# SrikarK-code/clip-dplm

Measured on AMD Instinct MI355X. Metric: seq-pairs/sec/node, contrastive training step, ESM-2-35M dual encoder, higher is better.
Workload: dtype bf16

## Files before the change

### clip_dplm_amd/_ffi.py

```python
from __future__ import annotations

import ctypes as C
import os

_HERE = os.path.dirname(os.path.abspath(__file__))
LIB_PATH = os.path.join(_HERE, "lib", "libclipk.so")

BF16, F32, U8 = 0, 1, 2
SAME_CLASS = {"mask": 0, "positive": 1}
ACT_NONE, ACT_RELU, ACT_GELU, ACT_CELU, ACT_SOFTPLUS = 0, 1, 2, 3, 4
ACT = {None: ACT_NONE, "none": ACT_NONE, "relu": ACT_RELU, "gelu": ACT_GELU, "celu": ACT_CELU, "softplus": ACT_SOFTPLUS}


class ClipkError(RuntimeError):
    pass


class GemmArgs(C.Structure):
    _fields_ = [
        ("A", C.c_void_p), ("lda", C.c_int64),
        ("B", C.c_void_p), ("ldb", C.c_int64),
        ("C", C.c_void_p), ("ldc", C.c_int64), ("c_dtype", C.c_int),
        ("M", C.c_int), ("N", C.c_int), ("K", C.c_int),
        ("bias", C.c_void_p),
        ("act", C.c_int),
        ("out_preact", C.c_void_p), ("ldp", C.c_int64),
        ("dact_aux", C.c_void_p), ("ldd", C.c_int64),
        ("dact", C.c_int),
        ("residual", C.c_void_p), ("ldr", C.c_int64), ("r_dtype", C.c_int),
        ("alpha", C.c_float),
        ("drop_p", C.c_float), ("drop_seed", C.c_uint32),
        ("rope_cos", C.c_void_p), ("rope_sin", C.c_void_p),
        ("rope_L", C.c_int), ("rope_hd", C.c_int), ("rope_cols", C.c_int), ("rope_row0", C.c_int),
        ("aux_dtype", C.c_int),
        ("rope_interleaved", C.c_int),
    ]


_vp, _i, _i64, _f, _sz = C.c_void_p, C.c_int, C.c_int64, C.c_float, C.c_size_t

SIGNATURES = {
    "clipk_version": (_i, []),
    "clipk_arch": (C.c_char_p, []),
    "clipk_status_string": (C.c_char_p, [_i]),
    "clipk_set_option": (_i, [C.c_char_p, _i]),
    "clipk_get_option": (_i, [C.c_char_p, C.POINTER(_i)]),
    "clipk_reset_options": (_i, []),
    "clipk_gemm_nt": (_i, [C.POINTER(GemmArgs), _vp]),
    "clipk_gemm_wgrad_workspace": (_sz, [_i, _i, _i]),
    "clipk_gemm_wgrad": (_i, [_vp, _i64, _vp, _i64, _vp, _i64, _vp, _i, _i, _i, _i, _i, _i, _vp, _sz, _vp]),
    "clipk_simce_workspace": (_sz, [_i, _i, _i]),
    "clipk_simce_lse": (_i, [_vp, _i, _vp, _i, _vp, _i, _i, _vp, _i, _vp, _vp, _vp, _sz, _vp]),
    "clipk_simce_grad": (_i, [_vp, _i, _vp, _i, _vp, _i, _i, _vp, _i, _vp, _vp, _f, _f, _f, _vp, _vp, _vp, _sz, _vp]),
    "clipk_simce_grad_scaled": (_i, [_vp, _i, _vp, _i, _vp, _i, _i, _vp, _i, _vp, _vp, _f, _f, _f, _vp, _vp, _vp, _vp, _sz, _vp]),
    "clipk_ce_combine": (_i, [_vp, _vp, _vp, _vp, _i, _f, _f, _f, _vp, _vp]),
    "clipk_simce_cls_workspace": (_sz, [_i, _i, _i]),
    "clipk_simce_lse_cls": (_i, [_vp, _i, _vp, _i, _vp, _i, _i, _vp, _i, _vp, _vp, _i, _f, _vp, _vp, _vp, _vp, _sz, _vp]),
    "clipk_simce_grad_cls": (_i, [_vp, _i, _vp, _i, _vp, _i, _i, _vp, _i, _vp, _vp, _vp, _vp, _vp, _vp, _i, _f, _i, _f, _f,
                                  _f, _vp, _vp, _vp, _vp, _sz, _vp]),
    "clipk_simce_hard_workspace": (_sz, [_i, _i, _i]),
    "clipk_simce_lse_hard": (_i, [_vp, _i, _vp, _i, _vp, _i, _i, _vp, _f, _i, _vp, _vp, _vp, _vp, _vp, _vp, _sz, _vp]),
    "clipk_simce_grad_hard": (_i, [_vp, _i, _vp, _i, _vp, _i, _i, _vp, _f, _i, _vp, _vp, _vp, _vp, _f, _f, _f, _vp, _vp,
                                   _vp, _vp, _sz, _vp]),
    "clipk_simce_pairs_workspace": (_sz, [_i, _i, _i]),
    "clipk_simce_lse_pairs": (_i, [_vp, _i, _i, _i, C.POINTER(_i), _i, _vp, _vp, _vp, _vp, _sz, _vp]),
    "clipk_simce_grad_pairs": (_i, [_vp, _i, _i, _i, C.POINTER(_i), C.POINTER(_i), _i, _vp, _vp, _f, _f, _f, _vp, _vp,
                                    _vp, _sz, _vp]),
    "clipk_simce_pairs_cls_workspace": (_sz, [_i, _i, _i]),
    "clipk_simce_lse_pairs_cls": (_i, [_vp, _i, _i, _i, C.POINTER(_i), _i, _vp, C.POINTER(_vp), _i, _f, _vp, _vp, _vp, _vp,
                                       _sz, _vp]),
    "clipk_simce_grad_pairs_cls": (_i, [_vp, _i, _i, _i, C.POINTER(_i), C.POINTER(_i), _i, _vp, C.POINTER(_vp), _i, _f, _vp,
                                        _vp, _f, _f, _f, _vp, _vp, _vp, _vp, _sz, _vp]),
    "clipk_simce_pairs_hard_workspace": (_sz, [_i, _i, _i]),
    "clipk_simce_lse_pairs_hard": (_i, [_vp, _i, _i, _i, C.POINTER(_i), _i, _vp, _f, C.POINTER(_vp), _vp, _vp, _vp, _vp,
                                        _sz, _vp]),
    "clipk_simce_grad_pairs_hard": (_i, [_vp, _i, _i, _i, C.POINTER(_i), C.POINTER(_i), _i, _vp, _f, C.POINTER(_vp), _vp,
                                         _f, _f, _f, _vp, _vp, _vp, _vp, _sz, _vp]),
    "clipk_sim_logits": (_i, [_vp, _i, _vp, _i, _i, _vp, _vp, _i64, _vp]),
    "clipk_sim_topk_workspace": (_sz, [_i, _i, _i, _i]),
    "clipk_sim_topk": (_i, [_vp, _i, _vp, _i, _i, _f, _i, _vp, _vp, _vp, _sz, _vp]),
    "clipk_sim_knn_workspace": (_sz, [_i, _i, _i, _i]),
    "clipk_sim_knn": (_i, [_vp, _i, _vp, _i, _i, _f, _vp, _i64, _vp, _vp, _i, _vp, _vp, _vp, _sz, _vp]),
# ... 140 lines not shown
```

### clip_dplm_amd/csrc/common.h

```cpp
#pragma once
#include <hip/hip_runtime.h>
#include <stdint.h>
#include "../../include/clipk.h"

#define CLIPK_ABI_VERSION 7
#define WAVE 64

enum clipk_opt {
  OPT_GEMM_KERNEL = 0,
  OPT_GEMM_EPI_GENERIC,
  OPT_GEMM_BM,
  OPT_GEMM_STAGES,
  OPT_GEMM_NWG,
  OPT_GEMM_STAGGER,
  OPT_EPI_NT,
  OPT_WGRAD_KERNEL,
  OPT_ATTN_WHOLE_FWD,
  OPT_ATTN_FUSED_BWD,
  OPT_ATTN_FUSED_WAVES,
  OPT_WGRAD_SPLITS,
  OPT_SIMCE_KERNEL,
  OPT_ATTN_ROW_STORES,
  OPT_GEMM_F32_SPLITS,
  OPT_RETRIEVAL_SPLITS,
  OPT_COUNT
};
int clipk_opt_get(int which);

typedef __attribute__((ext_vector_type(8))) short bf16x8;
typedef __attribute__((ext_vector_type(4))) short bf16x4;
typedef __attribute__((ext_vector_type(4))) float f32x4;
typedef __attribute__((ext_vector_type(16))) float f32x16;
typedef __attribute__((ext_vector_type(4))) unsigned int u32x4;
typedef __attribute__((ext_vector_type(2))) unsigned int u32x2;

__device__ __forceinline__ float bf16_to_f32(unsigned short h) {
  return __uint_as_float(((unsigned int)h) << 16);
}
__device__ __forceinline__ unsigned short f32_to_bf16(float f) {
  __bf16 b = (__bf16)f;
  return __builtin_bit_cast(unsigned short, b);
}
__device__ __forceinline__ unsigned int pack_bf16x2(float lo, float hi) {
  typedef __attribute__((ext_vector_type(2))) float v2f;
  typedef __attribute__((ext_vector_type(2))) __bf16 v2b;
  const v2b v = __builtin_convertvector(v2f{lo, hi}, v2b);
  return __builtin_bit_cast(unsigned int, v);
}

__device__ __forceinline__ void gelu_parts(float x, float& erf_abs, float& e) {
  const float ax = fabsf(x);
  const float t = __builtin_amdgcn_rcpf(fmaf(0.3275911f * 0.70710678118654752440f, ax, 1.0f));
  e = __builtin_amdgcn_exp2f(-0.72134752044448170368f * x * x);
  float poly = fmaf(1.061405429f, t, -1.453152027f);
  poly = fmaf(poly, t, 1.421413741f);
  poly = fmaf(poly, t, -0.284496736f);
  poly = fmaf(poly, t, 0.254829592f);
// ... 197 lines not shown
```

### clip_dplm_amd/csrc/core.hip

```cpp
#include "common.h"

extern "C" int clipk_version(void) { return CLIPK_ABI_VERSION; }
extern "C" const char* clipk_arch(void) { return "gfx950"; }
extern "C" const char* clipk_status_string(int status) {
  switch (status) {
    case CLIPK_OK: return "ok";
    case CLIPK_ERR_BAD_ARG: return "bad argument (null / misaligned pointer or non-positive dimension)";
    case CLIPK_ERR_UNSUPPORTED: return "unsupported shape for the gfx950 kernels";
    case CLIPK_ERR_LAUNCH: return "HIP launch error";
    default: return "unknown clipk status";
  }
}

#include <atomic>
#include <string.h>
namespace {
struct OptDef { const char* name; int dflt; };
const OptDef kOpts[OPT_COUNT] = {
    {"gemm_kernel", -1}, {"gemm_epi_generic", 0}, {"gemm_bm", 0}, {"gemm_stages", 1}, {"gemm_nwg", 0},
    {"gemm_stagger", 0}, {"epi_nt", 0}, {"wgrad_kernel", -1}, {"attn_whole_fwd", -1}, {"attn_fused_bwd", -1},
    {"attn_fused_waves", 0}, {"wgrad_splits", 0}, {"simce_kernel", -1},
    {"attn_row_stores", 0}, {"gemm_f32_splits", 0}, {"retrieval_splits", 0},
};
std::atomic<int> g_opts[OPT_COUNT];
std::atomic<bool> g_opts_init{false};
void opts_init() {
  if (!g_opts_init.load(std::memory_order_acquire)) {
    for (int i = 0; i < OPT_COUNT; ++i) g_opts[i].store(kOpts[i].dflt, std::memory_order_relaxed);
    g_opts_init.store(true, std::memory_order_release);
  }
}
int opt_index(const char* name) {
  if (!name) return -1;
  for (int i = 0; i < OPT_COUNT; ++i)
    if (strcmp(name, kOpts[i].name) == 0) return i;
  return -1;
}
}

namespace { std::atomic<const unsigned*> g_drop_epoch{nullptr}; }
const unsigned* clipk_drop_epoch() { return g_drop_epoch.load(std::memory_order_relaxed); }
extern "C" int clipk_set_dropout_epoch(const uint32_t* epoch_dev) {
  g_drop_epoch.store(reinterpret_cast<const unsigned*>(epoch_dev), std::memory_order_relaxed);
  return CLIPK_OK;
}

int clipk_opt_get(int which) {
  opts_init();
  return g_opts[which].load(std::memory_order_relaxed);
}
extern "C" int clipk_set_option(const char* name, int value) {
  opts_init();
  const int i = opt_index(name);
  if (i < 0) return CLIPK_ERR_BAD_ARG;
  g_opts[i].store(value, std::memory_order_relaxed);
// ... 15 lines not shown
```

### clip_dplm_amd/csrc/gemm_wgrad.hip

```cpp
#include "common.h"
#include <stdlib.h>

struct clipk_wgrad_v3_args {
  const unsigned short* dY; long lddy;
  const unsigned short* X; long ldx;
  float* slab; float* bslab;
  int M, N, K;
  int ntn, ntk, splits, m_per_split;
};
extern "C" void clipk_wgrad_v3_plan(int M, int N, int K, int* ntn, int* ntk, int* splits, int* mps);
extern "C" int clipk_wgrad_v3_launch(const clipk_wgrad_v3_args* a, void* stream);

namespace {

constexpr int BN = 128, BKO = 128, BMS = 64, NTHREADS = 256;
constexpr int ROWB = 256;
constexpr int TILE_BYTES = BMS * ROWB;
constexpr int LDS_BYTES = 2 * TILE_BYTES;

struct WP {
  const unsigned short* dY; long lddy;
  const unsigned short* X; long ldx;
  float* slab;
  float* bslab;
  int M, N, K;
  int ntn, ntk, splits, m_per_split;
};

typedef __attribute__((ext_vector_type(4))) short s16x4;

__device__ __forceinline__ int seg_off(int row, int seg) { return row * ROWB + ((seg ^ (row & 7)) << 5); }

__device__ __forceinline__ bf16x8 tr_frag(const char* tile, int row0, int seg, int pbyte) {
  const s16x4 lo = __builtin_amdgcn_ds_read_tr16_b64_v4i16(
      (s16x4 __attribute__((address_space(3)))*)(tile + seg_off(row0, seg) + pbyte));
  const s16x4 hi = __builtin_amdgcn_ds_read_tr16_b64_v4i16(
      (s16x4 __attribute__((address_space(3)))*)(tile + seg_off(row0 + 16, seg) + pbyte));
  bf16x8 f;
  f[0] = lo[0]; f[1] = lo[1]; f[2] = lo[2]; f[3] = lo[3];
  f[4] = hi[0]; f[5] = hi[1]; f[6] = hi[2]; f[7] = hi[3];
  return f;
}

// ... 88 lines not shown
      }
      if (do_bias) {
#pragma unroll
        for (int i = 0; i < 4; ++i) accb[i] = __builtin_amdgcn_mfma_f32_16x16x32_bf16(af[i], ones, accb[i], 0, 0, 0);
      }
    }
    __syncthreads();
  }

  float* slab = p.slab + (long)split * p.N * p.K;
#pragma unroll
  for (int i = 0; i < 4; ++i)
#pragma unroll
    for (int j = 0; j < 4; ++j) {
      const int k = k0 + wk * 64 + j * 16 + li;
#pragma unroll
      for (int r = 0; r < 4; ++r) {
        const int n = n0 + wn * 64 + i * 16 + 4 * g + r;
        if (n < p.N && k < p.K) slab[(long)n * p.K + k] = acc[i][j][r];
      }
    }
  if (do_bias && li == 0) {
#pragma unroll
    for (int i = 0; i < 4; ++i)
#pragma unroll
      for (int r = 0; r < 4; ++r) {
        const int n = n0 + wn * 64 + i * 16 + 4 * g + r;
        if (n < p.N) p.bslab[(long)split * p.N + n] = accb[i][r];
      }
  }
}

__global__ void wgrad_reduce_kernel(const float* slab, const float* bslab, int splits, int bsplits, int N, int K,
                                    float* dW, long lddw, float* dbias, int accumulate, int il_hd, int il_rows) {
  const long total4 = (long)N * K / 4;
  const int k4 = K >> 2;
  const long stride = (long)gridDim.x * blockDim.x;
  for (long i = blockIdx.x * (long)blockDim.x + threadIdx.x; i < total4; i += stride) {
    f32x4 a = f32x4{0.f, 0.f, 0.f, 0.f};
    const long sstride = (long)N * K / 4;
    const f32x4* src = reinterpret_cast<const f32x4*>(slab) + i;
    int s = 0;
    for (; s + 8 <= splits; s += 8) {
      f32x4 v[8];
#pragma unroll
      for (int e = 0; e < 8; ++e) v[e] = src[(long)(s + e) * sstride];
      a += (v[0] + v[1]) + (v[2] + v[3]);
      a += (v[4] + v[5]) + (v[6] + v[7]);
    }
    for (; s + 4 <= splits; s += 4) {
      const f32x4 v0 = src[(long)s * sstride], v1 = src[(long)(s + 1) * sstride];
      const f32x4 v2 = src[(long)(s + 2) * sstride], v3 = src[(long)(s + 3) * sstride];
      a += (v0 + v1) + (v2 + v3);
    }
    for (; s < splits; ++s) a += src[(long)s * sstride];
    const long n = i / k4; const int c = (int)(i - n * k4);
    f32x4* o = reinterpret_cast<f32x4*>(dW + (long)il_src((int)n, il_hd, il_rows) * lddw + 4 * c);
    *o = accumulate ? (*o + a) : a;
  }
  if (dbias) {
    for (long i = blockIdx.x * (long)blockDim.x + threadIdx.x; i < N; i += stride) {
      float a = 0.f;
      int s = 0;
      for (; s + 8 <= bsplits; s += 8) {
        float t[8];
#pragma unroll
        for (int e = 0; e < 8; ++e) t[e] = bslab[(long)(s + e) * N + i];
        a += ((t[0] + t[1]) + (t[2] + t[3])) + ((t[4] + t[5]) + (t[6] + t[7]));
      }
      for (; s < bsplits; ++s) a += bslab[(long)s * N + i];
      const int o = il_src((int)i, il_hd, il_rows);
      dbias[o] = accumulate ? dbias[o] + a : a;
    }
  }
}

struct Plan { int ntn, ntk, splits, mps; };
Plan make_plan(int M, int N, int K) {
  Plan pl;
  pl.ntn = (N + BN - 1) / BN; pl.ntk = (K + BKO - 1) / BKO;
  const int ntiles = pl.ntn * pl.ntk;
  int splits = (1024 + ntiles - 1) / ntiles;
  const int max_splits = (M + 8 * BMS - 1) / (8 * BMS);
  if (splits > max_splits) splits = max_splits;
  if (splits < 1) splits = 1;
  int mps = (M + splits - 1) / splits;
  mps = (mps + BMS - 1) / BMS * BMS;
  pl.mps = mps;
  pl.splits = (M + mps - 1) / mps;
  return pl;
}

bool use_v3(int M, int N, int K) {
  const int mode = clipk_opt_get(OPT_WGRAD_KERNEL);
  if (mode == 2) return false;
  if (mode == 3 || mode == 4) return M >= 1024;
  return M >= 16384 && N >= 128 && K >= 128;
}

}

extern "C" size_t clipk_gemm_wgrad_workspace(int M, int N, int K) {
  if (M <= 0 || N <= 0 || K <= 0) return 0;
  const Plan pl = make_plan(M, N, K);
  int ntn, ntk, splits, mps;
  clipk_wgrad_v3_plan(M, N, K, &ntn, &ntk, &splits, &mps);
  const size_t a = (size_t)pl.splits * ((size_t)N * K + N), b = (size_t)splits * ((size_t)N * K + (size_t)ntk * N);
  return (a > b ? a : b) * sizeof(float);
}

extern "C" int clipk_gemm_wgrad(const void* dY, int64_t lddy, const void* X, int64_t ldx,
                                float* dW, int64_t lddw, float* dbias, int M, int N, int K, int accumulate,
                                int il_hd, int il_rows, void* workspace, size_t workspace_bytes, void* stream) {
  if (!dY || !X || !dW || !workspace || M <= 0 || N <= 0 || K <= 0) return CLIPK_ERR_BAD_ARG;
  if (il_rows < 0 || il_rows > N || (il_rows > 0 && (il_hd < 2 || (il_hd & 1) || il_rows % il_hd))) return CLIPK_ERR_BAD_ARG;
  if (il_rows == 0) il_hd = 2;
  if ((N & 7) || (K & 7) || (lddy & 7) || (ldx & 7) || (lddw & 3)) return CLIPK_ERR_UNSUPPORTED;
  if (!aligned16(dY) || !aligned16(X) || !aligned16(dW) || !aligned16(workspace)) return CLIPK_ERR_BAD_ARG;
  hipStream_t st = (hipStream_t)stream;
  if (use_v3(M, N, K)) {
    clipk_wgrad_v3_args a;
    clipk_wgrad_v3_plan(M, N, K, &a.ntn, &a.ntk, &a.splits, &a.m_per_split);
    if (workspace_bytes < (size_t)a.splits * ((size_t)N * K + (size_t)a.ntk * N) * sizeof(float)) return CLIPK_ERR_BAD_ARG;
    a.dY = (const unsigned short*)dY; a.lddy = lddy;
    a.X = (const unsigned short*)X; a.ldx = ldx;
    a.slab = (float*)workspace;
    a.bslab = dbias ? (float*)workspace + (size_t)a.splits * N * K : nullptr;
    a.M = M; a.N = N; a.K = K;
    int rc = clipk_wgrad_v3_launch(&a, stream);
    if (rc) return rc;
    long total4 = (long)N * K / 4;
    int blocks = (int)((total4 + 255) / 256); if (blocks > 2048) blocks = 2048; if (blocks < 1) blocks = 1;
    hipLaunchKernelGGL(wgrad_reduce_kernel, dim3(blocks), dim3(256), 0, st, (const float*)a.slab, (const float*)a.bslab,
                       a.splits, a.splits * a.ntk, N, K, dW, (long)lddw, dbias, accumulate, il_hd, il_rows);
    return clipk_check_launch();
  }
  const Plan pl = make_plan(M, N, K);
  const size_t need = (size_t)pl.splits * ((size_t)N * K + N) * sizeof(float);
  if (workspace_bytes < need) return CLIPK_ERR_BAD_ARG;
  WP p;
  p.dY = (const unsigned short*)dY; p.lddy = lddy;
  p.X = (const unsigned short*)X; p.ldx = ldx;
  p.slab = (float*)workspace;
  p.bslab = dbias ? (float*)workspace + (size_t)pl.splits * N * K : nullptr;
  p.M = M; p.N = N; p.K = K;
  p.ntn = pl.ntn; p.ntk = pl.ntk; p.splits = pl.splits; p.m_per_split = pl.mps;
  hipLaunchKernelGGL(wgrad_kernel, dim3(pl.ntn * pl.ntk * pl.splits), dim3(NTHREADS), LDS_BYTES, st, p);
  int rc = clipk_check_launch();
  if (rc) return rc;
  long total4 = (long)N * K / 4;
  int blocks = (int)((total4 + 255) / 256); if (blocks > 2048) blocks = 2048; if (blocks < 1) blocks = 1;
  hipLaunchKernelGGL(wgrad_reduce_kernel, dim3(blocks), dim3(256), 0, st, (const float*)p.slab, (const float*)p.bslab,
                     pl.splits, pl.splits, N, K, dW, (long)lddw, dbias, accumulate, il_hd, il_rows);
  return clipk_check_launch();
}
```

### clip_dplm_amd/csrc/gemm_wgrad_v3.hip

```cpp
#include "common.h"
#include <stdlib.h>
#include <type_traits>

struct clipk_wgrad_v3_args {
  const unsigned short* dY; long lddy;
  const unsigned short* X; long ldx;
  float* slab;
  float* bslab;
  int M, N, K;
  int ntn, ntk, splits, m_per_split;
};

namespace {

constexpr int BN = 256, BKO = 256, BMS = 64;
constexpr int ROWB = 256;
constexpr int HALF_BYTES = BMS * ROWB;
constexpr int BUF_BYTES = 4 * HALF_BYTES;
constexpr int LDS_BYTES = 2 * BUF_BYTES;
constexpr int YH0 = 0, YH1 = HALF_BYTES, XH0 = 2 * HALF_BYTES, XH1 = 3 * HALF_BYTES;

typedef __attribute__((ext_vector_type(2))) unsigned int u32x2;

template <int OFF>
__device__ __forceinline__ u32x2 ds_tr16(unsigned lds_addr) {
  u32x2 v;
  asm volatile("ds_read_b64_tr_b16 %0, %1 offset:%2" : "=v"(v) : "v"(lds_addr), "n"(OFF));
  return v;
}
template <int OFF>
__device__ __forceinline__ bf16x8 tr_pair(unsigned lds_addr) {
  const u32x2 lo = ds_tr16<OFF>(lds_addr);
  const u32x2 hi = ds_tr16<OFF + 16 * ROWB>(lds_addr);
  const u32x4 f = {lo[0], lo[1], hi[0], hi[1]};
  return __builtin_bit_cast(bf16x8, f);
}

template <int KH, int NH>
__device__ __forceinline__ void quad(f32x4 (&acc)[8][4], const bf16x8 (&yf)[4][2], const bf16x8 (&xf)[2][2][2]) {
#pragma unroll
  for (int ms = 0; ms < 2; ++ms)
#pragma unroll
    for (int u = 0; u < 2; ++u)
#pragma unroll
      for (int t = 0; t < 4; ++t)
        acc[NH * 4 + t][KH * 2 + u] =
            __builtin_amdgcn_mfma_f32_16x16x32_bf16(yf[t][ms], xf[KH][u][ms], acc[NH * 4 + t][KH * 2 + u], 0, 0, 0);
}

#define CLIPK_SB() __builtin_amdgcn_sched_barrier(0)
#define CLIPK_BAR() __builtin_amdgcn_s_barrier()

template <int SCHED>
__global__ __launch_bounds__(512, 1) void wgrad_v3_kernel(const clipk_wgrad_v3_args p) {
  extern __shared__ __attribute__((aligned(16))) char smem[];
  const int tid = threadIdx.x, lane = tid & 63;
  const int wid = __builtin_amdgcn_readfirstlane(tid >> 6);
  const int wn = wid >> 2, wk = wid & 3;
  const int ntiles = p.ntn * p.ntk;
  const int bid = xcd_remap(blockIdx.x, gridDim.x);
  const int split = bid / ntiles;
  const int tile = bid - split * ntiles;
  const int tn = tile / p.ntk, tk = tile - tn * p.ntk;
  const int n0 = tn * BN, k0 = tk * BKO;
  const int M = p.M, N = p.N, K = p.K;
  const int m_beg = split * p.m_per_split;
  int m_end = m_beg + p.m_per_split; m_end = m_end < M ? m_end : M;
  const int nkt = (m_end - m_beg + BMS - 1) / BMS;
  const bool has_bias = p.bslab != nullptr;
  int bias_T = tk;

  unsigned yv[2], xv[2];
#pragma unroll
  for (int i = 0; i < 2; ++i) {
    const int row = 4 * (2 * wid + i) + (lane >> 4);
    const int slot = lane & 15;
    const int col = (((slot >> 1) ^ (row & 7)) << 4) + (slot & 1) * 8;
    yv[i] = (unsigned)(((long)row * p.lddy + (col >> 6) * 128 + (col & 63)) * 2);
    xv[i] = (unsigned)(((long)row * p.ldx + (col >> 5) * 64 + (col & 31)) * 2);
  }
  const unsigned short* y_end = p.dY + ((long)(M - 1) * p.lddy + N);
  const unsigned short* x_end = p.X + ((long)(M - 1) * p.ldx + K);
  auto stage = [&](bool is_y, int half, int T, int region) {
    const long mt = (long)m_beg + (long)T * BMS;
    const unsigned short* base = is_y ? p.dY + mt * p.lddy + (n0 + half * 64) : p.X + mt * p.ldx + (k0 + half * 32);
    const long left = ((is_y ? y_end : x_end) - base) * 2;
    const int bytes = left > 0 ? (int)(left < 0x7fffffffL ? left : 0x7fffffffL) : 0;
    const auto d = __builtin_amdgcn_make_buffer_rsrc((void*)base, 0, bytes, 0x00020000);
    char* dst = smem + (T & 1) * BUF_BYTES + region + wid * 2048;
#pragma unroll
    for (int i = 0; i < 2; ++i)
      __builtin_amdgcn_raw_ptr_buffer_load_lds(d, (__attribute__((address_space(3))) void*)(dst + i * 1024), 16,
                                               (int)(is_y ? yv[i] : xv[i]), 0, 0, 0);
  };
  auto stage1 = [&](bool is_y, int half, int T, int region, int i) {
    const long mt = (long)m_beg + (long)T * BMS;
    const unsigned short* base = is_y ? p.dY + mt * p.lddy + (n0 + half * 64) : p.X + mt * p.ldx + (k0 + half * 32);
    const long left = ((is_y ? y_end : x_end) - base) * 2;
    const int bytes = left > 0 ? (int)(left < 0x7fffffffL ? left : 0x7fffffffL) : 0;
    const auto d = __builtin_amdgcn_make_buffer_rsrc((void*)base, 0, bytes, 0x00020000);
    char* dst = smem + (T & 1) * BUF_BYTES + region + wid * 2048 + i * 1024;
    __builtin_amdgcn_raw_ptr_buffer_load_lds(d, (__attribute__((address_space(3))) void*)dst, 16,
                                             (int)(is_y ? (i ? yv[1] : yv[0]) : (i ? xv[1] : xv[0])), 0, 0, 0);
  };

  f32x4 acc[8][4];
#pragma unroll
  for (int i = 0; i < 8; ++i)
#pragma unroll
    for (int j = 0; j < 4; ++j) acc[i][j] = f32x4{0.f, 0.f, 0.f, 0.f};
  f32x4 accb[2][2];
#pragma unroll
  for (int u = 0; u < 2; ++u) { accb[u][0] = f32x4{0.f, 0.f, 0.f, 0.f}; accb[u][1] = accb[u][0]; }
  bf16x8 ones;
#pragma unroll
  for (int j = 0; j < 8; ++j) ones[j] = (short)0x3F80;

  const int g = lane >> 4, li = lane & 15;
  const int trow = 4 * g + (li >> 2);
  const int sw = trow & 7;
  const unsigned lds0 = (unsigned)(size_t)(__attribute__((address_space(3))) char*)smem;
  unsigned ya[4], xa[2];
#pragma unroll
  for (int t = 0; t < 4; ++t) ya[t] = lds0 + trow * ROWB + (((wn * 4 + t) ^ sw) << 5) + 8 * (li & 3);
#pragma unroll
  for (int u = 0; u < 2; ++u) xa[u] = lds0 + trow * ROWB + (((wk * 2 + u) ^ sw) << 5) + 8 * (li & 3);

  if constexpr (SCHED == 1) {
    bf16x8 yf[4][2], xf[2][2][2];

// ... 76 lines not shown
      CLIPK_SB();
      __builtin_amdgcn_s_setprio(1);
      quad<1, 1>(acc, yf, xf);
      __builtin_amdgcn_s_setprio(0);
      CLIPK_SB(); CLIPK_BAR(); CLIPK_SB();
      if (TM == 0) {
        stage(false, 1, T + 2, XH1);
        asm volatile("s_waitcnt vmcnt(6)" ::: "memory");
      } else if (TM == 1) {
        asm volatile("s_waitcnt vmcnt(0)" ::: "memory");
      }
      CLIPK_SB(); CLIPK_BAR(); CLIPK_SB();
      __builtin_amdgcn_s_setprio(1);
      quad<0, 1>(acc, yf, xf);
      if (bias_now) { bias_tile(accb[1][0], accb[1][1]); bias_T += p.ntk; }
      __builtin_amdgcn_s_setprio(0);
      CLIPK_SB(); CLIPK_BAR(); CLIPK_SB();
    };

    stage(false, 0, 0, XH0); stage(true, 0, 0, YH0); stage(false, 1, 0, XH1); stage(true, 1, 0, YH1);
    if (nkt > 1) {
      stage(false, 0, 1, XH0); stage(true, 0, 1, YH0); stage(false, 1, 1, XH1);
      asm volatile("s_waitcnt vmcnt(6)" ::: "memory");
    } else {
      asm volatile("s_waitcnt vmcnt(0)" ::: "memory");
    }
    CLIPK_SB(); CLIPK_BAR(); CLIPK_SB();
    if (wn == 1) CLIPK_BAR();
    for (int T = 0; T < nkt - 2; ++T) step_body(std::integral_constant<int, 0>{}, T);
    if (nkt > 1) step_body(std::integral_constant<int, 1>{}, nkt - 2);
    step_body(std::integral_constant<int, 2>{}, nkt - 1);
    if (wn == 0) CLIPK_BAR();
  } else {
    bf16x8 yq[2][2][2], xf[2][2][2];
    auto read_yq = [&](auto q_c, unsigned bo) {
      constexpr int q = decltype(q_c)::value;
      constexpr int REG = (q >> 1) ? YH1 : YH0;
#pragma unroll
      for (int t = 0; t < 2; ++t) {
        yq[q & 1][t][0] = tr_pair<REG>(ya[(q & 1) * 2 + t] + bo);
        yq[q & 1][t][1] = tr_pair<REG + 32 * ROWB>(ya[(q & 1) * 2 + t] + bo);
      }
    };
    auto read_x = [&](auto kh_c, unsigned bo) {
      constexpr int kh = decltype(kh_c)::value;
      constexpr int REG = kh ? XH1 : XH0;
#pragma unroll
      for (int u = 0; u < 2; ++u) {
        xf[kh][u][0] = tr_pair<REG>(xa[u] + bo);
        xf[kh][u][1] = tr_pair<REG + 32 * ROWB>(xa[u] + bo);
      }
    };
    auto blk = [&](auto kh_c, auto q_c, auto&& mid) {
      constexpr int kh = decltype(kh_c)::value, q = decltype(q_c)::value;
#pragma unroll
      for (int ms = 0; ms < 2; ++ms) {
#pragma unroll
        for (int u = 0; u < 2; ++u)
#pragma unroll
          for (int t = 0; t < 2; ++t)
            acc[q * 2 + t][kh * 2 + u] = __builtin_amdgcn_mfma_f32_16x16x32_bf16(yq[q & 1][t][ms], xf[kh][u][ms],
                                                                                 acc[q * 2 + t][kh * 2 + u], 0, 0, 0);
        if (ms == 0) { CLIPK_SB(); mid(); CLIPK_SB(); }
      }
    };
    const int b_odd = wk >> 1, b_sel = wk & 1;
    auto bias_mfma = [](int odd, int sel, int qo, f32x4& a0, f32x4& a1, const bf16x8& on, const bf16x8& y00,
                        const bf16x8& y01, const bf16x8& y10, const bf16x8& y11) {
      asm volatile(
          "s_nop 1\n\t"
          "s_cmp_lg_u32 %[odd], %[qo]\n\t"
          "s_cbranch_scc1 2f\n\t"
          "s_cmp_lg_u32 %[sel], 0\n\t"
          "s_cbranch_scc1 1f\n\t"
          "v_mfma_f32_16x16x32_bf16 %[a0], %[y00], %[on], %[a0]\n\t"
          "v_mfma_f32_16x16x32_bf16 %[a1], %[y01], %[on], %[a1]\n\t"
          "s_branch 2f\n"
          "1:\n\t"
          "v_mfma_f32_16x16x32_bf16 %[a0], %[y10], %[on], %[a0]\n\t"
          "v_mfma_f32_16x16x32_bf16 %[a1], %[y11], %[on], %[a1]\n"
          "2:\n\t"
          : [a0] "+v"(a0), [a1] "+v"(a1)
          : [odd] "s"(odd), [sel] "s"(sel), [qo] "s"(qo), [on] "v"(on), [y00] "v"(y00), [y01] "v"(y01),
            [y10] "v"(y10), [y11] "v"(y11)
          : "scc");
    };
#define CLIPK_BIAS_Q(q, a0, a1) \
  bias_mfma(b_odd, b_sel, (q) & 1, a0, a1, ones, yq[(q) & 1][0][0], yq[(q) & 1][0][1], yq[(q) & 1][1][0], yq[(q) & 1][1][1])
    using I0 = std::integral_constant<int, 0>; using I1 = std::integral_constant<int, 1>;
    using I2 = std::integral_constant<int, 2>; using I3 = std::integral_constant<int, 3>;
#define CLIPK_LGKM0() asm volatile("s_waitcnt lgkmcnt(0)" ::: "memory")

    auto step2 = [&](auto mode_c, int T) {
      constexpr int TM = decltype(mode_c)::value;
      const unsigned bo = (T & 1) * BUF_BYTES, bn = ((T + 1) & 1) * BUF_BYTES;
      const bool bias_now = has_bias && T == bias_T;
      const bool y1_next = TM != 2 && T >= 1;
      auto none = [] {};
      CLIPK_LGKM0(); CLIPK_SB();
      read_yq(I1{}, bo); read_x(I1{}, bo);
      CLIPK_SB();
      blk(I0{}, I0{}, [&] { if (y1_next) stage1(true, 1, T + 1, YH1, 0); });
      if (bias_now) CLIPK_BIAS_Q(0, accb[0][0], accb[0][1]);
      CLIPK_SB();
      CLIPK_LGKM0(); CLIPK_SB();
      blk(I1{}, I0{}, [&] { if (y1_next) stage1(true, 1, T + 1, YH1, 1); });
      CLIPK_SB();
      if (TM == 2) asm volatile("s_waitcnt vmcnt(0)" ::: "memory");
      else asm volatile("s_waitcnt vmcnt(8)" ::: "memory");
      CLIPK_SB(); CLIPK_BAR(); CLIPK_SB();
      read_yq(I2{}, bo);
      CLIPK_SB();
      blk(I1{}, I1{}, [&] { if (TM == 0) stage1(true, 0, T + 2, YH0, 0); });
      if (bias_now) CLIPK_BIAS_Q(1, accb[0][0], accb[0][1]);
      CLIPK_SB();
      blk(I0{}, I1{}, [&] { if (TM == 0) stage1(true, 0, T + 2, YH0, 1); });
      CLIPK_SB();
      CLIPK_LGKM0(); CLIPK_SB();
      read_yq(I3{}, bo);
      CLIPK_SB();
      blk(I0{}, I2{}, [&] { if (TM == 0) stage1(false, 0, T + 2, XH0, 0); });
      if (bias_now) CLIPK_BIAS_Q(2, accb[1][0], accb[1][1]);
      CLIPK_SB();
      blk(I1{}, I2{}, [&] { if (TM == 0) stage1(false, 0, T + 2, XH0, 1); });
      CLIPK_SB();
      CLIPK_LGKM0();
      if (TM == 0) asm volatile("s_waitcnt vmcnt(6)" ::: "memory");
      else if (TM == 1) asm volatile("s_waitcnt vmcnt(2)" ::: "memory");
      CLIPK_SB(); CLIPK_BAR(); CLIPK_SB();
      if (TM != 2) read_yq(I0{}, bn);
      CLIPK_SB();
      blk(I0{}, I3{}, [&] { if (TM == 0) stage1(false, 1, T + 2, XH1, 0); });
      if (bias_now) CLIPK_BIAS_Q(3, accb[1][0], accb[1][1]);
      CLIPK_SB();
      if (TM != 2) read_x(I0{}, bn);
      CLIPK_SB();
      blk(I1{}, I3{}, [&] { if (TM == 0) stage1(false, 1, T + 2, XH1, 1); });
      if (bias_now) bias_T += p.ntk;
      CLIPK_SB();
      (void)none;
    };

    stage(true, 0, 0, YH0); stage(false, 0, 0, XH0); stage(false, 1, 0, XH1); stage(true, 1, 0, YH1);
    if (nkt > 1) {
      stage(true, 0, 1, YH0); stage(false, 0, 1, XH0); stage(false, 1, 1, XH1); stage(true, 1, 1, YH1);
      asm volatile("s_waitcnt vmcnt(8)" ::: "memory");
    } else {
      asm volatile("s_waitcnt vmcnt(0)" ::: "memory");
    }
    CLIPK_SB(); CLIPK_BAR(); CLIPK_SB();
    read_yq(I0{}, 0u); read_x(I0{}, 0u);
    for (int T = 0; T < nkt - 2; ++T) step2(std::integral_constant<int, 0>{}, T);
    if (nkt > 1) step2(std::integral_constant<int, 1>{}, nkt - 2);
    step2(std::integral_constant<int, 2>{}, nkt - 1);
  }

  float* slab = p.slab + (long)split * N * K;
#pragma unroll
  for (int i = 0; i < 8; ++i)
#pragma unroll
    for (int r = 0; r < 4; ++r) {
      const int n = n0 + wn * 128 + i * 16 + 4 * g + r;
#pragma unroll
      for (int j = 0; j < 4; ++j) {
        const int k = k0 + wk * 64 + j * 16 + li;
        if (n < N && k < K) slab[(long)n * K + k] = acc[i][j][r];
      }
    }
  if (has_bias && li == 0) {
    float* bs = p.bslab + ((long)split * p.ntk + tk) * N;
#pragma unroll
    for (int u = 0; u < 2; ++u)
#pragma unroll
      for (int r = 0; r < 4; ++r) {
        const int n = n0 + wn * 128 + u * 64 + wk * 16 + 4 * g + r;
        if (n < N) bs[n] = accb[u][0][r] + accb[u][1][r];
      }
  }
}

}

extern "C" void clipk_wgrad_v3_plan(int M, int N, int K, int* ntn, int* ntk, int* splits, int* mps) {
  *ntn = (N + BN - 1) / BN; *ntk = (K + BKO - 1) / BKO;
  const int ntiles = *ntn * *ntk;
  int s = 256 / ntiles;
  if (clipk_opt_get(OPT_WGRAD_SPLITS) > 0) s = clipk_opt_get(OPT_WGRAD_SPLITS);
  if (s < 1) s = 1;
  const int max_splits = (M + 8 * BMS - 1) / (8 * BMS);
  if (s > max_splits) s = max_splits;
  int m = (M + s - 1) / s;
  m = (m + BMS - 1) / BMS * BMS;
  *mps = m;
  *splits = (M + m - 1) / m;
}

extern "C" int clipk_wgrad_v3_launch(const clipk_wgrad_v3_args* a, void* stream) {
  static std::atomic<uint64_t> attr_set{0};
  clipk_once_per_device(attr_set, [&] {
    (void)hipFuncSetAttribute(reinterpret_cast<const void*>(wgrad_v3_kernel<1>),
                              hipFuncAttributeMaxDynamicSharedMemorySize, LDS_BYTES);
    (void)hipFuncSetAttribute(reinterpret_cast<const void*>(wgrad_v3_kernel<2>),
                              hipFuncAttributeMaxDynamicSharedMemorySize, LDS_BYTES);
  });
  const dim3 grid(a->ntn * a->ntk * a->splits);
  if (clipk_opt_get(OPT_WGRAD_KERNEL) == 3)
    hipLaunchKernelGGL(wgrad_v3_kernel<1>, grid, dim3(512), LDS_BYTES, (hipStream_t)stream, *a);
  else
    hipLaunchKernelGGL(wgrad_v3_kernel<2>, grid, dim3(512), LDS_BYTES, (hipStream_t)stream, *a);
  return clipk_check_launch();
}
```

### include/clipk.h

```cpp
#ifndef CLIPK_H
#define CLIPK_H

#include <stddef.h>
#include <stdint.h>

#ifdef __cplusplus
extern "C" {
#endif

typedef enum clipk_status {
  CLIPK_OK = 0,
  CLIPK_ERR_BAD_ARG = -1,
  CLIPK_ERR_UNSUPPORTED = -2,
  CLIPK_ERR_LAUNCH = -3
} clipk_status;

typedef enum clipk_dtype { CLIPK_BF16 = 0, CLIPK_F32 = 1, CLIPK_U8 = 2 } clipk_dtype;
typedef enum clipk_act { CLIPK_ACT_NONE = 0, CLIPK_ACT_RELU = 1, CLIPK_ACT_GELU = 2, CLIPK_ACT_CELU = 3,
                         CLIPK_ACT_SOFTPLUS = 4 } clipk_act;

int clipk_version(void);
const char* clipk_arch(void);
const char* clipk_status_string(int status);

int clipk_set_option(const char* name, int value);
int clipk_get_option(const char* name, int* value);
int clipk_reset_options(void);

typedef struct clipk_gemm_args {
  const void* A; int64_t lda;
  const void* B; int64_t ldb;
  void* C; int64_t ldc; int c_dtype;
  int M, N, K;
  const float* bias;
  int act;
  void* out_preact; int64_t ldp;
  const void* dact_aux; int64_t ldd;
  int dact;
  const void* residual; int64_t ldr; int r_dtype;
  float alpha;
  float drop_p; uint32_t drop_seed;
  const float* rope_cos; const float* rope_sin; int rope_L, rope_hd, rope_cols, rope_row0;
  int aux_dtype;
  int rope_interleaved;
} clipk_gemm_args;
int clipk_gemm_nt(const clipk_gemm_args* args, void* stream);

size_t clipk_gemm_wgrad_workspace(int M, int N, int K);
int clipk_gemm_wgrad(const void* dY, int64_t lddy, const void* X, int64_t ldx,
                     float* dW, int64_t lddw, float* dbias,
                     int M, int N, int K, int accumulate, int il_hd, int il_rows,
                     void* workspace, size_t workspace_bytes, void* stream);

size_t clipk_simce_workspace(int Mx, int Nkeys, int P);
int clipk_simce_lse(const float* X, int Mx, const float* Y, int Ny, const float* Yc, int Nc,
                    int P, const float* scale ,
                    int label_offset, float* lse , float* pos ,
                    void* workspace, size_t workspace_bytes, void* stream);

int clipk_simce_grad(const float* X, int Mx, const float* Y, int Ny, const float* Yc, int Nc,
                     int P, const float* scale, int label_offset,
                     const float* lse_x, const float* lse_y, float w_row, float w_col, float inv_bg,
                     float* dX , float* dscale_partial ,
                     void* workspace, size_t workspace_bytes, void* stream);
int clipk_simce_grad_scaled(const float* X, int Mx, const float* Y, int Ny, const float* Yc, int Nc,
                            int P, const float* scale, int label_offset,
                            const float* lse_x, const float* lse_y, float w_row, float w_col, float inv_bg,
                            const float* upstream, float* dX , float* dscale_partial ,
                            void* workspace, size_t workspace_bytes, void* stream);
int clipk_ce_combine(const float* lse_r, const float* pos_r, const float* lse_c, const float* pos_c, int n,
                     float w_row, float w_col, float bg, float* loss, void* stream);

enum { CLIPK_SAME_CLASS_MASK = 0, CLIPK_SAME_CLASS_POSITIVE = 1 };
size_t clipk_simce_cls_workspace(int Mx, int Nkeys, int P);
int clipk_simce_lse_cls(const float* X, int Mx, const float* Y, int Ny, const float* Yc, int Nc, int P,
                        const float* scale, int label_offset, const int64_t* cls_x, const int64_t* cls_y,
                        int same_class, float eps, float* lse , float* tgt , float* cnt ,
                        void* workspace, size_t workspace_bytes, void* stream);
int clipk_simce_grad_cls(const float* X, int Mx, const float* Y, int Ny, const float* Yc, int Nc, int P,
                         const float* scale, int label_offset, const float* lse_x, const float* lse_y,
                         const float* cnt_x, const float* cnt_y, const int64_t* cls_x, const int64_t* cls_y,
                         int same_class, float eps, int nkeys_y, float w_row, float w_col, float inv_bg,
                         const float* upstream, float* dX , float* dscale_partial ,
                         void* workspace, size_t workspace_bytes, void* stream);

// ... 311 lines not shown
```

Before: 6504.

## Weight ragged last N-tile in wgrad v3 split planning and skip dead MFMAs

```diff
diff --git a/clip_dplm_amd/_ffi.py b/clip_dplm_amd/_ffi.py
--- a/clip_dplm_amd/_ffi.py
+++ b/clip_dplm_amd/_ffi.py
@@ -48,6 +48,7 @@
     "clipk_reset_options": (_i, []),
     "clipk_gemm_nt": (_i, [C.POINTER(GemmArgs), _vp]),
     "clipk_gemm_wgrad_workspace": (_sz, [_i, _i, _i]),
+    "clipk_gemm_wgrad_plan": (None, [_i, _i, _i, _i, _i, _i, C.POINTER(_i)]),
     "clipk_gemm_wgrad": (_i, [_vp, _i64, _vp, _i64, _vp, _i64, _vp, _i, _i, _i, _i, _i, _i, _vp, _sz, _vp]),
     "clipk_simce_workspace": (_sz, [_i, _i, _i]),
     "clipk_simce_lse": (_i, [_vp, _i, _vp, _i, _vp, _i, _i, _vp, _i, _vp, _vp, _vp, _sz, _vp]),
diff --git a/clip_dplm_amd/csrc/common.h b/clip_dplm_amd/csrc/common.h
--- a/clip_dplm_amd/csrc/common.h
+++ b/clip_dplm_amd/csrc/common.h
@@ -23,6 +23,8 @@
   OPT_ATTN_ROW_STORES,
   OPT_GEMM_F32_SPLITS,
   OPT_RETRIEVAL_SPLITS,
+  OPT_WGRAD_PLAN,
+  OPT_WGRAD_GROUPS,
   OPT_COUNT
 };
 int clipk_opt_get(int which);
diff --git a/clip_dplm_amd/csrc/core.hip b/clip_dplm_amd/csrc/core.hip
--- a/clip_dplm_amd/csrc/core.hip
+++ b/clip_dplm_amd/csrc/core.hip
@@ -21,6 +21,7 @@
     {"gemm_stagger", 0}, {"epi_nt", 0}, {"wgrad_kernel", -1}, {"attn_whole_fwd", -1}, {"attn_fused_bwd", -1},
     {"attn_fused_waves", 0}, {"wgrad_splits", 0}, {"simce_kernel", -1},
     {"attn_row_stores", 0}, {"gemm_f32_splits", 0}, {"retrieval_splits", 0},
+    {"wgrad_plan", 0}, {"wgrad_groups", 0},
 };
 std::atomic<int> g_opts[OPT_COUNT];
 std::atomic<bool> g_opts_init{false};
diff --git a/clip_dplm_amd/csrc/gemm_wgrad.hip b/clip_dplm_amd/csrc/gemm_wgrad.hip
--- a/clip_dplm_amd/csrc/gemm_wgrad.hip
+++ b/clip_dplm_amd/csrc/gemm_wgrad.hip
@@ -7,8 +7,11 @@
   float* slab; float* bslab;
   int M, N, K;
   int ntn, ntk, splits, m_per_split;
+  int live, splits_l, m_per_split_l;
 };
-extern "C" void clipk_wgrad_v3_plan(int M, int N, int K, int* ntn, int* ntk, int* splits, int* mps);
+struct clipk_wgrad_v3_plan_t { int ntn, ntk, splits, mps, live, splits_l, mps_l; };
+extern "C" void clipk_wgrad_v3_plan(int M, int N, int K, clipk_wgrad_v3_plan_t* pl);
+extern "C" void clipk_wgrad_v3_plan_pure(int M, int N, int K, int G, int force_splits, int uniform, clipk_wgrad_v3_plan_t* pl);
 extern "C" int clipk_wgrad_v3_launch(const clipk_wgrad_v3_args* a, void* stream);
 
 namespace {
@@ -163,7 +166,8 @@
 }
 
 __global__ void wgrad_reduce_kernel(const float* slab, const float* bslab, int splits, int bsplits, int N, int K,
-                                    float* dW, long lddw, float* dbias, int accumulate, int il_hd, int il_rows) {
+                                    float* dW, long lddw, float* dbias, int accumulate, int il_hd, int il_rows,
+                                    int n_last, int splits_l, int bsplits_l) {
   const long total4 = (long)N * K / 4;
   const int k4 = K >> 2;
   const long stride = (long)gridDim.x * blockDim.x;
@@ -171,35 +175,37 @@
     f32x4 a = f32x4{0.f, 0.f, 0.f, 0.f};
     const long sstride = (long)N * K / 4;
     const f32x4* src = reinterpret_cast<const f32x4*>(slab) + i;
+    const long n = i / k4; const int c = (int)(i - n * k4);
+    const int nsp = n >= n_last ? splits_l : splits;
     int s = 0;
-    for (; s + 8 <= splits; s += 8) {
+    for (; s + 8 <= nsp; s += 8) {
       f32x4 v[8];
 #pragma unroll
       for (int e = 0; e < 8; ++e) v[e] = src[(long)(s + e) * sstride];
       a += (v[0] + v[1]) + (v[2] + v[3]);
       a += (v[4] + v[5]) + (v[6] + v[7]);
     }
-    for (; s + 4 <= splits; s += 4) {
+    for (; s + 4 <= nsp; s += 4) {
       const f32x4 v0 = src[(long)s * sstride], v1 = src[(long)(s + 1) * sstride];
       const f32x4 v2 = src[(long)(s + 2) * sstride], v3 = src[(long)(s + 3) * sstride];
       a += (v0 + v1) + (v2 + v3);
     }
-    for (; s < splits; ++s) a += src[(long)s * sstride];
-    const long n = i / k4; const int c = (int)(i - n * k4);
+    for (; s < nsp; ++s) a += src[(long)s * sstride];
     f32x4* o = reinterpret_cast<f32x4*>(dW + (long)il_src((int)n, il_hd, il_rows) * lddw + 4 * c);
     *o = accumulate ? (*o + a) : a;
   }
   if (dbias) {
     for (long i = blockIdx.x * (long)blockDim.x + threadIdx.x; i < N; i += stride) {
       float a = 0.f;
+      const int nbs = i >= n_last ? bsplits_l : bsplits;
       int s = 0;
-      for (; s + 8 <= bsplits; s += 8) {
+      for (; s + 8 <= nbs; s += 8) {
         float t[8];
 #pragma unroll
         for (int e = 0; e < 8; ++e) t[e] = bslab[(long)(s + e) * N + i];
         a += ((t[0] + t[1]) + (t[2] + t[3])) + ((t[4] + t[5]) + (t[6] + t[7]));
       }
-      for (; s < bsplits; ++s) a += bslab[(long)s * N + i];
+      for (; s < nbs; ++s) a += bslab[(long)s * N + i];
       const int o = il_src((int)i, il_hd, il_rows);
       dbias[o] = accumulate ? dbias[o] + a : a;
     }
@@ -231,12 +237,19 @@
 
 }
 
+extern "C" void clipk_gemm_wgrad_plan(int M, int N, int K, int groups, int force_splits, int uniform, int* out) {
+  clipk_wgrad_v3_plan_t pl;
+  clipk_wgrad_v3_plan_pure(M, N, K, groups, force_splits, uniform, &pl);
+  out[0] = pl.ntn; out[1] = pl.ntk; out[2] = pl.splits; out[3] = pl.mps; out[4] = pl.live; out[5] = pl.splits_l; out[6] = pl.mps_l;
+}
+
 extern "C" size_t clipk_gemm_wgrad_workspace(int M, int N, int K) {
   if (M <= 0 || N <= 0 || K <= 0) return 0;
   const Plan pl = make_plan(M, N, K);
-  int ntn, ntk, splits, mps;
-  clipk_wgrad_v3_plan(M, N, K, &ntn, &ntk, &splits, &mps);
-  const size_t a = (size_t)pl.splits * ((size_t)N * K + N), b = (size_t)splits * ((size_t)N * K + (size_t)ntk * N);
+  clipk_wgrad_v3_plan_t p3;
+  clipk_wgrad_v3_plan(M, N, K, &p3);
+  const int slabs = p3.splits > p3.splits_l ? p3.splits : p3.splits_l;
+  const size_t a = (size_t)pl.splits * ((size_t)N * K + N), b = (size_t)slabs * ((size_t)N * K + (size_t)p3.ntk * N);
   return (a > b ? a : b) * sizeof(float);
 }
 
@@ -251,19 +264,25 @@
   hipStream_t st = (hipStream_t)stream;
   if (use_v3(M, N, K)) {
     clipk_wgrad_v3_args a;
-    clipk_wgrad_v3_plan(M, N, K, &a.ntn, &a.ntk, &a.splits, &a.m_per_split);
-    if (workspace_bytes < (size_t)a.splits * ((size_t)N * K + (size_t)a.ntk * N) * sizeof(float)) return CLIPK_ERR_BAD_ARG;
+    clipk_wgrad_v3_plan_t p3;
+    clipk_wgrad_v3_plan(M, N, K, &p3);
+    a.ntn = p3.ntn; a.ntk = p3.ntk; a.splits = p3.splits; a.m_per_split = p3.mps;
+    a.live = p3.live; a.splits_l = p3.splits_l; a.m_per_split_l = p3.mps_l;
+    const int slabs = a.splits > a.splits_l ? a.splits : a.splits_l;
+    const int n_last = a.live > 0 ? (a.ntn - 1) * 256 : N;
+    if (workspace_bytes < (size_t)slabs * ((size_t)N * K + (size_t)a.ntk * N) * sizeof(float)) return CLIPK_ERR_BAD_ARG;
     a.dY = (const unsigned short*)dY; a.lddy = lddy;
     a.X = (const unsigned short*)X; a.ldx = ldx;
     a.slab = (float*)workspace;
-    a.bslab = dbias ? (float*)workspace + (size_t)a.splits * N * K : nullptr;
+    a.bslab = dbias ? (float*)workspace + (size_t)slabs * N * K : nullptr;
     a.M = M; a.N = N; a.K = K;
     int rc = clipk_wgrad_v3_launch(&a, stream);
     if (rc) return rc;
     long total4 = (long)N * K / 4;
     int blocks = (int)((total4 + 255) / 256); if (blocks > 2048) blocks = 2048; if (blocks < 1) blocks = 1;
     hipLaunchKernelGGL(wgrad_reduce_kernel, dim3(blocks), dim3(256), 0, st, (const float*)a.slab, (const float*)a.bslab,
-                       a.splits, a.splits * a.ntk, N, K, dW, (long)lddw, dbias, accumulate, il_hd, il_rows);
+                       a.splits, a.splits * a.ntk, N, K, dW, (long)lddw, dbias, accumulate, il_hd, il_rows, n_last,
+                       a.splits_l, a.splits_l * a.ntk);
     return clipk_check_launch();
   }
   const Plan pl = make_plan(M, N, K);
@@ -282,6 +301,6 @@
   long total4 = (long)N * K / 4;
   int blocks = (int)((total4 + 255) / 256); if (blocks > 2048) blocks = 2048; if (blocks < 1) blocks = 1;
   hipLaunchKernelGGL(wgrad_reduce_kernel, dim3(blocks), dim3(256), 0, st, (const float*)p.slab, (const float*)p.bslab,
-                     pl.splits, pl.splits, N, K, dW, (long)lddw, dbias, accumulate, il_hd, il_rows);
+                     pl.splits, pl.splits, N, K, dW, (long)lddw, dbias, accumulate, il_hd, il_rows, N, 0, 0);
   return clipk_check_launch();
 }
diff --git a/clip_dplm_amd/csrc/gemm_wgrad_v3.hip b/clip_dplm_amd/csrc/gemm_wgrad_v3.hip
--- a/clip_dplm_amd/csrc/gemm_wgrad_v3.hip
+++ b/clip_dplm_amd/csrc/gemm_wgrad_v3.hip
@@ -9,7 +9,9 @@
   float* bslab;
   int M, N, K;
   int ntn, ntk, splits, m_per_split;
+  int live, splits_l, m_per_split_l;
 };
+struct clipk_wgrad_v3_plan_t { int ntn, ntk, splits, mps, live, splits_l, mps_l; };
 
 namespace {
 
@@ -51,7 +53,7 @@
 #define CLIPK_SB() __builtin_amdgcn_sched_barrier(0)
 #define CLIPK_BAR() __builtin_amdgcn_s_barrier()
 
-template <int SCHED>
+template <int SCHED, int LIVE>
 __global__ __launch_bounds__(512, 1) void wgrad_v3_kernel(const clipk_wgrad_v3_args p) {
   extern __shared__ __attribute__((aligned(16))) char smem[];
   const int tid = threadIdx.x, lane = tid & 63;
@@ -59,13 +61,20 @@
   const int wn = wid >> 2, wk = wid & 3;
   const int ntiles = p.ntn * p.ntk;
   const int bid = xcd_remap(blockIdx.x, gridDim.x);
-  const int split = bid / ntiles;
-  const int tile = bid - split * ntiles;
+  const bool deal = p.live > 0;
+  const int nfull = LIVE < 8 ? ntiles - p.ntk : ntiles;
+  int split, tile, mps;
+  if (bid < nfull * p.splits) {
+    split = bid / nfull; tile = bid - split * nfull; mps = p.m_per_split;
+  } else {
+    const int b2 = bid - nfull * p.splits;
+    split = b2 / p.ntk; tile = nfull + (b2 - split * p.ntk); mps = p.m_per_split_l;
+  }
   const int tn = tile / p.ntk, tk = tile - tn * p.ntk;
   const int n0 = tn * BN, k0 = tk * BKO;
   const int M = p.M, N = p.N, K = p.K;
-  const int m_beg = split * p.m_per_split;
-  int m_end = m_beg + p.m_per_split; m_end = m_end < M ? m_end : M;
+  const int m_beg = split * mps;
+  int m_end = m_beg + mps; m_end = m_end < M ? m_end : M;
   const int nkt = (m_end - m_beg + BMS - 1) / BMS;
   const bool has_bias = p.bslab != nullptr;
   int bias_T = tk;
@@ -76,14 +85,16 @@
     const int row = 4 * (2 * wid + i) + (lane >> 4);
     const int slot = lane & 15;
     const int col = (((slot >> 1) ^ (row & 7)) << 4) + (slot & 1) * 8;
-    yv[i] = (unsigned)(((long)row * p.lddy + (col >> 6) * 128 + (col & 63)) * 2);
+    const int ycol = deal ? ((col >> 4) & 3) * 32 + (col >> 6) * 16 + (col & 15) : (col >> 6) * 128 + (col & 63);
+    yv[i] = (unsigned)(((long)row * p.lddy + ycol) * 2);
     xv[i] = (unsigned)(((long)row * p.ldx + (col >> 5) * 64 + (col & 31)) * 2);
   }
+  const int yhalf = deal ? 128 : 64;
   const unsigned short* y_end = p.dY + ((long)(M - 1) * p.lddy + N);
   const unsigned short* x_end = p.X + ((long)(M - 1) * p.ldx + K);
   auto stage = [&](bool is_y, int half, int T, int region) {
     const long mt = (long)m_beg + (long)T * BMS;
-    const unsigned short* base = is_y ? p.dY + mt * p.lddy + (n0 + half * 64) : p.X + mt * p.ldx + (k0 + half * 32);
+    const unsigned short* base = is_y ? p.dY + mt * p.lddy + (n0 + half * yhalf) : p.X + mt * p.ldx + (k0 + half * 32);
     const long left = ((is_y ? y_end : x_end) - base) * 2;
     const int bytes = left > 0 ? (int)(left < 0x7fffffffL ? left : 0x7fffffffL) : 0;
     const auto d = __builtin_amdgcn_make_buffer_rsrc((void*)base, 0, bytes, 0x00020000);
@@ -95,7 +106,7 @@
   };
   auto stage1 = [&](bool is_y, int half, int T, int region, int i) {
     const long mt = (long)m_beg + (long)T * BMS;
-    const unsigned short* base = is_y ? p.dY + mt * p.lddy + (n0 + half * 64) : p.X + mt * p.ldx + (k0 + half * 32);
+    const unsigned short* base = is_y ? p.dY + mt * p.lddy + (n0 + half * yhalf) : p.X + mt * p.ldx + (k0 + half * 32);
     const long left = ((is_y ? y_end : x_end) - base) * 2;
     const int bytes = left > 0 ? (int)(left < 0x7fffffffL ? left : 0x7fffffffL) : 0;
     const auto d = __builtin_amdgcn_make_buffer_rsrc((void*)base, 0, bytes, 0x00020000);
@@ -238,12 +249,15 @@
     step_body(std::integral_constant<int, 2>{}, nkt - 1);
     if (wn == 0) CLIPK_BAR();
   } else {
+    auto run2 = [&](auto live_c) {
+    constexpr int LV = decltype(live_c)::value;
     bf16x8 yq[2][2][2], xf[2][2][2];
     auto read_yq = [&](auto q_c, unsigned bo) {
       constexpr int q = decltype(q_c)::value;
       constexpr int REG = (q >> 1) ? YH1 : YH0;
 #pragma unroll
       for (int t = 0; t < 2; ++t) {
+        if (2 * q + t >= LV) continue;
         yq[q & 1][t][0] = tr_pair<REG>(ya[(q & 1) * 2 + t] + bo);
         yq[q & 1][t][1] = tr_pair<REG + 32 * ROWB>(ya[(q & 1) * 2 + t] + bo);
       }
@@ -265,8 +279,9 @@
         for (int u = 0; u < 2; ++u)
 #pragma unroll
           for (int t = 0; t < 2; ++t)
-            acc[q * 2 + t][kh * 2 + u] = __builtin_amdgcn_mfma_f32_16x16x32_bf16(yq[q & 1][t][ms], xf[kh][u][ms],
-                                                                                 acc[q * 2 + t][kh * 2 + u], 0, 0, 0);
+            if (q * 2 + t < LV)
+              acc[q * 2 + t][kh * 2 + u] = __builtin_amdgcn_mfma_f32_16x16x32_bf16(yq[q & 1][t][ms], xf[kh][u][ms],
+                                                                                   acc[q * 2 + t][kh * 2 + u], 0, 0, 0);
         if (ms == 0) { CLIPK_SB(); mid(); CLIPK_SB(); }
       }
     };
@@ -291,8 +306,13 @@
             [y10] "v"(y10), [y11] "v"(y11)
           : "scc");
     };
-#define CLIPK_BIAS_Q(q, a0, a1) \
-  bias_mfma(b_odd, b_sel, (q) & 1, a0, a1, ones, yq[(q) & 1][0][0], yq[(q) & 1][0][1], yq[(q) & 1][1][0], yq[(q) & 1][1][1])
+#define CLIPK_BIAS_Q(q, a0, a1)                                                                                       \
+  do {                                                                                                                \
+    constexpr int t1_ = 2 * (q) + 1 < LV ? 1 : 0;      \
+    if constexpr (2 * (q) < LV)                                                                                       \
+      bias_mfma(b_odd, b_sel, (q) & 1, a0, a1, ones, yq[(q) & 1][0][0], yq[(q) & 1][0][1], yq[(q) & 1][t1_][0],       \
+                yq[(q) & 1][t1_][1]);                                                                                 \
+  } while (0)
     using I0 = std::integral_constant<int, 0>; using I1 = std::integral_constant<int, 1>;
     using I2 = std::integral_constant<int, 2>; using I3 = std::integral_constant<int, 3>;
 #define CLIPK_LGKM0() asm volatile("s_waitcnt lgkmcnt(0)" ::: "memory")
@@ -359,6 +379,13 @@
     for (int T = 0; T < nkt - 2; ++T) step2(std::integral_constant<int, 0>{}, T);
     if (nkt > 1) step2(std::integral_constant<int, 1>{}, nkt - 2);
     step2(std::integral_constant<int, 2>{}, nkt - 1);
+    };
+    if constexpr (LIVE < 8) {
+      if (tn == p.ntn - 1) run2(std::integral_constant<int, LIVE>{});
+      else run2(std::integral_constant<int, 8>{});
+    } else {
+      run2(std::integral_constant<int, 8>{});
+    }
   }
 
   float* slab = p.slab + (long)split * N * K;
@@ -366,7 +393,7 @@
   for (int i = 0; i < 8; ++i)
 #pragma unroll
     for (int r = 0; r < 4; ++r) {
-      const int n = n0 + wn * 128 + i * 16 + 4 * g + r;
+      const int n = n0 + (deal ? i * 32 + wn * 16 : wn * 128 + i * 16) + 4 * g + r;
 #pragma unroll
       for (int j = 0; j < 4; ++j) {
         const int k = k0 + wk * 64 + j * 16 + li;
@@ -379,40 +406,93 @@
     for (int u = 0; u < 2; ++u)
 #pragma unroll
       for (int r = 0; r < 4; ++r) {
-        const int n = n0 + wn * 128 + u * 64 + wk * 16 + 4 * g + r;
+        const int n = n0 + (deal ? (4 * u + wk) * 32 + wn * 16 : wn * 128 + u * 64 + wk * 16) + 4 * g + r;
         if (n < N) bs[n] = accb[u][0][r] + accb[u][1][r];
       }
   }
 }
 
-}
-
-extern "C" void clipk_wgrad_v3_plan(int M, int N, int K, int* ntn, int* ntk, int* splits, int* mps) {
-  *ntn = (N + BN - 1) / BN; *ntk = (K + BKO - 1) / BKO;
-  const int ntiles = *ntn * *ntk;
-  int s = 256 / ntiles;
-  if (clipk_opt_get(OPT_WGRAD_SPLITS) > 0) s = clipk_opt_get(OPT_WGRAD_SPLITS);
-  if (s < 1) s = 1;
-  const int max_splits = (M + 8 * BMS - 1) / (8 * BMS);
-  if (s > max_splits) s = max_splits;
+int split_rows(int M, int s, int* mps) {
   int m = (M + s - 1) / s;
   m = (m + BMS - 1) / BMS * BMS;
   *mps = m;
-  *splits = (M + m - 1) / m;
+  return (M + m - 1) / m;
+}
+
+}
+
+extern "C" void clipk_wgrad_v3_plan_pure(int M, int N, int K, int G, int force_splits, int uniform,
+                                         clipk_wgrad_v3_plan_t* pl) {
+  pl->ntn = (N + BN - 1) / BN; pl->ntk = (K + BKO - 1) / BKO;
+  const int ntiles = pl->ntn * pl->ntk;
+  const int max_splits = (M + 8 * BMS - 1) / (8 * BMS);
+  const int nblocks = (N - (pl->ntn - 1) * BN + 15) / 16;
+  const int live = (nblocks + 1) / 2;
+  const int nf = ntiles - pl->ntk, nl = pl->ntk;
+  if (G < 1) G = 1;
+  if (force_splits > 0 || uniform || live >= 8 || nf + nl > G) {
+    int s = force_splits > 0 ? force_splits : G / ntiles;
+    if (s < 1) s = 1;
+    if (s > max_splits) s = max_splits;
+    pl->splits = split_rows(M, s, &pl->mps);
+    pl->live = 0; pl->splits_l = pl->splits; pl->mps_l = pl->mps;
+    return;
+  }
+  auto steps = [&](int s) { int m; (void)split_rows(M, s, &m); return m / BMS; };
+  auto cap = [&](int s) { return s < 1 ? 0 : (s > max_splits ? max_splits : s); };
+  int sf = 0, sl = cap(G / nl);
+  if (nf > 0) {
+    long best = -1;
+    const int sf_max = cap((G - nl) / nf);
+    for (int f = 1; f <= sf_max; ++f) {
+      const int l = cap((G - nf * f) / nl);
+      const long cf = (long)steps(f) * 8, cl = (long)steps(l) * live;
+      const long c = cf > cl ? cf : cl;
+      if (best < 0 || c < best) { best = c; sf = f; sl = l; }
+    }
+    while (sl > 1 && (long)steps(sl - 1) * live <= (long)steps(sf) * 8) --sl;
+  }
+  pl->live = live;
+  pl->splits_l = split_rows(M, sl, &pl->mps_l);
+  if (sf > 0) pl->splits = split_rows(M, sf, &pl->mps);
+  else { pl->splits = 0; pl->mps = pl->mps_l; }
+}
+
+extern "C" void clipk_wgrad_v3_plan(int M, int N, int K, clipk_wgrad_v3_plan_t* pl) {
+  const int groups = clipk_opt_get(OPT_WGRAD_GROUPS);
+  const int G = groups > 0 ? groups : clipk_cu_count();
+  const bool uniform = clipk_opt_get(OPT_WGRAD_PLAN) == 1 || clipk_opt_get(OPT_WGRAD_KERNEL) == 3;
+  clipk_wgrad_v3_plan_pure(M, N, K, G, clipk_opt_get(OPT_WGRAD_SPLITS), uniform, pl);
 }
 
 extern "C" int clipk_wgrad_v3_launch(const clipk_wgrad_v3_args* a, void* stream) {
   static std::atomic<uint64_t> attr_set{0};
   clipk_once_per_device(attr_set, [&] {
-    (void)hipFuncSetAttribute(reinterpret_cast<const void*>(wgrad_v3_kernel<1>),
-                              hipFuncAttributeMaxDynamicSharedMemorySize, LDS_BYTES);
-    (void)hipFuncSetAttribute(reinterpret_cast<const void*>(wgrad_v3_kernel<2>),
-                              hipFuncAttributeMaxDynamicSharedMemorySize, LDS_BYTES);
+    const void* k[] = {reinterpret_cast<const void*>(wgrad_v3_kernel<1, 8>), reinterpret_cast<const void*>(wgrad_v3_kernel<2, 8>),
+                       reinterpret_cast<const void*>(wgrad_v3_kernel<2, 1>), reinterpret_cast<const void*>(wgrad_v3_kernel<2, 2>),
+                       reinterpret_cast<const void*>(wgrad_v3_kernel<2, 3>), reinterpret_cast<const void*>(wgrad_v3_kernel<2, 4>),
+                       reinterpret_cast<const void*>(wgrad_v3_kernel<2, 5>), reinterpret_cast<const void*>(wgrad_v3_kernel<2, 6>),
+                       reinterpret_cast<const void*>(wgrad_v3_kernel<2, 7>)};
+    for (const void* f : k) (void)hipFuncSetAttribute(f, hipFuncAttributeMaxDynamicSharedMemorySize, LDS_BYTES);
   });
-  const dim3 grid(a->ntn * a->ntk * a->splits);
-  if (clipk_opt_get(OPT_WGRAD_KERNEL) == 3)
-    hipLaunchKernelGGL(wgrad_v3_kernel<1>, grid, dim3(512), LDS_BYTES, (hipStream_t)stream, *a);
-  else
-    hipLaunchKernelGGL(wgrad_v3_kernel<2>, grid, dim3(512), LDS_BYTES, (hipStream_t)stream, *a);
+  const bool weighted = a->live >= 1 && a->live < 8;
+  const int nfull = weighted ? (a->ntn - 1) * a->ntk : a->ntn * a->ntk;
+  const dim3 grid(nfull * a->splits + (weighted ? a->ntk * a->splits_l : 0)), block(512);
+  hipStream_t st = (hipStream_t)stream;
+  if (clipk_opt_get(OPT_WGRAD_KERNEL) == 3) {
+    if (a->live != 0) return CLIPK_ERR_BAD_ARG;
+    hipLaunchKernelGGL((wgrad_v3_kernel<1, 8>), grid, block, LDS_BYTES, st, *a);
+  } else {
+    switch (weighted ? a->live : 8) {
+      case 1: hipLaunchKernelGGL((wgrad_v3_kernel<2, 1>), grid, block, LDS_BYTES, st, *a); break;
+      case 2: hipLaunchKernelGGL((wgrad_v3_kernel<2, 2>), grid, block, LDS_BYTES, st, *a); break;
+      case 3: hipLaunchKernelGGL((wgrad_v3_kernel<2, 3>), grid, block, LDS_BYTES, st, *a); break;
+      case 4: hipLaunchKernelGGL((wgrad_v3_kernel<2, 4>), grid, block, LDS_BYTES, st, *a); break;
+      case 5: hipLaunchKernelGGL((wgrad_v3_kernel<2, 5>), grid, block, LDS_BYTES, st, *a); break;
+      case 6: hipLaunchKernelGGL((wgrad_v3_kernel<2, 6>), grid, block, LDS_BYTES, st, *a); break;
+      case 7: hipLaunchKernelGGL((wgrad_v3_kernel<2, 7>), grid, block, LDS_BYTES, st, *a); break;
+      default: hipLaunchKernelGGL((wgrad_v3_kernel<2, 8>), grid, block, LDS_BYTES, st, *a); break;
+    }
+  }
   return clipk_check_launch();
 }
diff --git a/include/clipk.h b/include/clipk.h
--- a/include/clipk.h
+++ b/include/clipk.h
@@ -51,6 +51,7 @@
                      float* dW, int64_t lddw, float* dbias,
                      int M, int N, int K, int accumulate, int il_hd, int il_rows,
                      void* workspace, size_t workspace_bytes, void* stream);
+void clipk_gemm_wgrad_plan(int M, int N, int K, int groups, int force_splits, int uniform, int* out);
 
 size_t clipk_simce_workspace(int Mx, int Nkeys, int P);
 int clipk_simce_lse(const float* X, int Mx, const float* Y, int Ny, const float* Yc, int Nc,
```

Result: slower. 6254 (-3.8%).
